# aiola-lab/whisper-medusa

Measured on AMD Instinct MI355X. Metric: decoded_tokens_per_sec, higher is better.
Workload: dtype bf16 + fp16 decoder GEMM operands (one plane; fp32 accumulate)

## Files before the change

### whisper-medusa_amd/csrc/wm_decoder.hip

```cpp
#include "wm_internal.h"
#include <algorithm>
#include <cstdlib>
#include <type_traits>
#include "wm_skinny_gemm.h"
#include "wm_select.h"

__global__ void k_embed(float* __restrict__ h, const bf16_t* __restrict__ tok_emb, const float* __restrict__ pos_emb,
                        const int* __restrict__ base, const int* __restrict__ tok_src, int tok_stride, int use_base_off,
                        int Mper, int d, int V, int Tmax, const int* __restrict__ depth,
                        const int4* __restrict__ rowinfo = nullptr, const int* __restrict__ ids = nullptr, int ids_stride = 0,
                        const float* __restrict__ gnext = nullptr, bf16_t* __restrict__ xo = nullptr, size_t xplane = 0,
                        float2* __restrict__ stats = nullptr, int sld = 0)
{
    const int row = blockIdx.x;
    int s = row / Mper, r = row - s * Mper;
    bool base_row = false;
    int b0;
    if (rowinfo) {
        const int4 ri = rowinfo[row];
        if (ri.w == 0) return;
        s = ri.x; r = ri.y; b0 = ri.z; base_row = ri.w == 1;
    } else {
        b0 = base[s];
    }
// ... 483 lines not shown
                ov[sp] = *reinterpret_cast<const float4*>(&s_part[spc][qr][ch]);
            }
        }
        float Mx = -INFINITY;
#pragma unroll
        for (int sp = 0; sp < WM_XATTN_NS_MAX; ++sp) if (sp < NS) Mx = fmaxf(Mx, ms[sp]);
        float Lt = 0.f; float4 o4 = make_float4(0.f, 0.f, 0.f, 0.f);
#pragma unroll
        for (int sp = 0; sp < WM_XATTN_NS_MAX; ++sp) {
            if (sp < NS) {
                const float e = (ms[sp] == -INFINITY) ? 0.f : __expf(ms[sp] - Mx);
                Lt += ls[sp] * e;
                o4.x += ov[sp].x * e; o4.y += ov[sp].y * e; o4.z += ov[sp].z * e; o4.w += ov[sp].w * e;
            }
        }
        const float inv = vsc / Lt;
        const size_t oi = packed_index(row, hd * 64 + ch, K32);
        act_st4(xout + oi, xout + xplane + oi, make_float4(o4.x * inv, o4.y * inv, o4.z * inv, o4.w * inv));
    }
    TL_END
}


__device__ __forceinline__ void sib_block_pop(float (&tv)[6], int (&ti)[6], float* sv, int* si, int tid, float& mx, int& mi)
{
    const int lane = tid & 63, w = tid >> 6;
    mx = tv[0]; mi = ti[0];
#pragma unroll
    for (int o = 32; o > 0; o >>= 1) {
        const float ov = __shfl_xor(mx, o, 64); const int oi = __shfl_xor(mi, o, 64);
        if (ov > mx || (ov == mx && oi < mi)) { mx = ov; mi = oi; }
    }
    __syncthreads();
    if (lane == 0) { sv[w] = mx; si[w] = mi; }
    __syncthreads();
    mx = sv[0]; mi = si[0];
#pragma unroll
    for (int q = 1; q < 4; ++q) if (sv[q] > mx || (sv[q] == mx && si[q] < mi)) { mx = sv[q]; mi = si[q]; }
    if (ti[0] == mi && mi != 0x7fffffff) {
#pragma unroll
        for (int q = 0; q < 5; ++q) { tv[q] = tv[q + 1]; ti[q] = ti[q + 1]; }
        tv[5] = -INFINITY; ti[5] = 0x7fffffff;
    }
}
__device__ __forceinline__ void sib_insert(float (&tv)[6], int (&ti)[6], float v, int vi)
{
    if (v > tv[5] || (v == tv[5] && vi < ti[5])) {
#pragma unroll
        for (int j = 0; j < 6; ++j)
            if (v > tv[j] || (v == tv[j] && vi < ti[j])) { const float fv = tv[j]; const int fi = ti[j]; tv[j] = v; ti[j] = vi; v = fv; vi = fi; }
    }
}

template <bool NEED_Z, bool TS>
__device__ __forceinline__ void
select1_body(const float* __restrict__ logits, const GenDev& gp, const unsigned char* __restrict__ mask, const float* __restrict__ exppen,
             const int* __restrict__ L, int rps, float* __restrict__ part1, const int4* __restrict__ rowinfo, float2* __restrict__ sibpart,
             const TsDev& ts, int ts_verify)
{
    __shared__ float sv[4]; __shared__ int si[4]; __shared__ float sz[4];
    const int row = blockIdx.y, sp = blockIdx.x;
    int s = row / rps, ri_i = row - s * rps;
    const bool sibrow = sibpart != nullptr && row - s * rps == 1;
    if (rowinfo) {
        const int4 ri = rowinfo[row];
        if (ri.w != 2) return;
        s = ri.x; ri_i = ri.y;
    }
    const int tid = threadIdx.x, lane = tid & 63, w = tid >> 6;
    const int cur_len = L[s];
    const float* x = logits + (size_t)row * gp.Vpad;
    const int per = (gp.V + SEL_SP - 1) / SEL_SP, n0 = sp * per, n1 = min(gp.V, n0 + per);
    int4 rec = make_int4(0, 0, 0, 0);
    if (TS) rec = ts_row_record(gp, ts, ts_verify, s, ri_i, cur_len);
    extern __shared__ unsigned rp_sh[];
    const bool rp = TS && ts.rp != 0;
    if (rp) rp_build(ts, rp_row_prefix(ts, ts_verify, s, ri_i, cur_len), n0, n1, -1, gp.V, rp_sh, tid, 256);
    auto pl = [&](int n) {
        float v = x[n];
        if (rp) v = rp_pen(v, n, n0, ts, rp_sh);
        v = proc_logit(v, n, cur_len, gp, mask, exppen);
        if (TS) v = ts_mask(v, n, rec, gp, ts);
        if (rp && rp_banned(n, n0, gp.V, rp_sh)) v = -INFINITY;
        return v;
    };
    float mx = -INFINITY; int mi = 0x7fffffff;
    if (sibrow) {
        float tv[6]; int ti[6];
#pragma unroll
        for (int j = 0; j < 6; ++j) { tv[j] = -INFINITY; ti[j] = 0x7fffffff; }
        for (int n = n0 + tid; n < n1; n += 256) sib_insert(tv, ti, pl(n), n);
        float2* mine = sibpart + ((size_t)s * SEL_SP + sp) * 6;
        float m0 = -INFINITY; int i0 = 0x7fffffff;
        for (int j = 0; j < 6; ++j) {
            float pm; int pi;
            sib_block_pop(tv, ti, sv, si, tid, pm, pi);
            if (j == 0) { m0 = pm; i0 = pi; }
            if (tid == 0) mine[j] = make_float2(pm, __int_as_float(pi));
        }
        __syncthreads();
        mx = m0; mi = i0;
    } else if (!TS) {
        for (int n = n0 + tid; n < n1; n += 256) {
            const float v = proc_logit(x[n], n, cur_len, gp, mask, exppen);
            if (v > mx || (v == mx && n < mi)) { mx = v; mi = n; }
        }
#pragma unroll
        for (int o = 32; o > 0; o >>= 1) {
            const float ov = __shfl_xor(mx, o, 64); const int oi = __shfl_xor(mi, o, 64);
            if (ov > mx || (ov == mx && oi < mi)) { mx = ov; mi = oi; }
        }
        if (lane == 0) { sv[w] = mx; si[w] = mi; }
        __syncthreads();
        mx = sv[0]; mi = si[0];
#pragma unroll
        for (int k = 1; k < 4; ++k) if (sv[k] > mx || (sv[k] == mx && si[k] < mi)) { mx = sv[k]; mi = si[k]; }
    }
    if (TS) {
        float mt = -INFINITY, ms = -INFINITY; int it = 0x7fffffff, is = 0x7fffffff;
        for (int n = n0 + tid; n < n1; n += 256) {
            const float v = pl(n);
            if (n < ts.tb) { if (v > mt || (v == mt && n < it)) { mt = v; it = n; } }
            else if (v > ms || (v == ms && n < is)) { ms = v; is = n; }
        }
        block_argmax(mt, it, sv, si, tid);
        block_argmax(ms, is, sv, si, tid);
        float zt = 0.f, zs = 0.f, zs1 = 0.f;
        for (int n = (NEED_Z ? n0 : max(n0, ts.tb)) + tid; n < n1; n += 256) {
            const float v = pl(n);
            if (v == -INFINITY) continue;
            if (n < ts.tb) zt += expf((v - mt) * gp.inv_temp);
            else { if (NEED_Z) zs += expf((v - ms) * gp.inv_temp); zs1 += expf(v - ms); }
        }
        zt = block_sum(zt, sz, tid); zs = block_sum(zs, sz, tid); zs1 = block_sum(zs1, sz, tid);
        if (tid == 0) {
            float* o = part1 + ((size_t)row * SEL_SP + sp) * 4;
            o[0] = mt; o[1] = __int_as_float(it); o[2] = zt;
            float* q = ts.part1t + ((size_t)row * SEL_SP + sp) * 4;
            q[0] = ms; q[1] = __int_as_float(is); q[2] = zs; q[3] = zs1;
        }
        return;
    }
    float z = 0.f;
    if (NEED_Z && mx != -INFINITY)
        for (int n = n0 + tid; n < n1; n += 256) {
            const float v = proc_logit(x[n], n, cur_len, gp, mask, exppen);
            z += (v == -INFINITY) ? 0.f : expf((v - mx) * gp.inv_temp);
        }
    z = wave_sum(z);
    if (lane == 0) sz[w] = z;
    __syncthreads();
    if (tid == 0) {
        float* o = part1 + ((size_t)row * SEL_SP + sp) * 4;
        o[0] = mx; o[1] = __int_as_float(mi); o[2] = (sz[0] + sz[1]) + (sz[2] + sz[3]);
    }
}

template <bool NEED_Z = true>
__global__ void __launch_bounds__(256)
k_select1(const float* __restrict__ logits, GenDev gp, const unsigned char* __restrict__ mask, const float* __restrict__ exppen,
          const int* __restrict__ L, int rps, float* __restrict__ part1, const int4* __restrict__ rowinfo = nullptr,
          float2* __restrict__ sibpart = nullptr)
{
    select1_body<NEED_Z, false>(logits, gp, mask, exppen, L, rps, part1, rowinfo, sibpart, TsDev{}, 0);
}
template <bool NEED_Z>
__global__ void __launch_bounds__(256)
k_select1_ts(const float* __restrict__ logits, GenDev gp, const unsigned char* __restrict__ mask, const float* __restrict__ exppen,
             const int* __restrict__ L, int rps, float* __restrict__ part1, const int4* __restrict__ rowinfo, float2* __restrict__ sibpart,
             TsDev ts, int ts_verify)
{
    select1_body<NEED_Z, true>(logits, gp, mask, exppen, L, rps, part1, rowinfo, sibpart, ts, ts_verify);
}

template <bool TS>
__device__ __forceinline__ void
select2_body(const float* __restrict__ logits, const GenDev& gp, const unsigned char* __restrict__ mask, const float* __restrict__ exppen,
             const int* __restrict__ L, const int* __restrict__ cand, int rps, int out_row0, const float* __restrict__ part1,
             float* __restrict__ part2, int* __restrict__ amax, float* __restrict__ pc, const TreeDev* __restrict__ tree,
             const int4* __restrict__ rowinfo, const TsDev& ts)
{
    __shared__ float sh[4];
    const int row = blockIdx.y, sp = blockIdx.x;
    int s = row / rps, i = row - s * rps;
    if (rowinfo) {
        const int4 ri = rowinfo[row];
        if (ri.w != 2) return;
        s = ri.x; i = ri.y;
    }
    const int tid = threadIdx.x, lane = tid & 63, w = tid >> 6;
    const int cur_len = L[s];
    const float* x = logits + (size_t)row * gp.Vpad;
    const float* p1 = part1 + (size_t)row * SEL_SP * 4;
    float mx = -INFINITY; int mi = 0x7fffffff;
    float invz;
    int4 rec = make_int4(0, 0, 0, 0); int forced = 0;
    if (TS) {
        const TsSel f = ts_finish(p1, ts.part1t + (size_t)row * SEL_SP * 4, gp.inv_temp);
        mx = f.mx; mi = f.mi; invz = 1.0f / f.z; forced = f.forced;
        rec = ts_row_record(gp, ts, 1, s, i, cur_len);
    } else {
#pragma unroll
        for (int k = 0; k < SEL_SP; ++k) {
            const float v = p1[4 * k]; const int idx = __float_as_int(p1[4 * k + 1]);
            if (v > mx || (v == mx && idx < mi)) { mx = v; mi = idx; }
        }
        float z = 0.f;
#pragma unroll
        for (int k = 0; k < SEL_SP; ++k) {
            const float v = p1[4 * k];
            z += (v == -INFINITY) ? 0.f : p1[4 * k + 2] * expf((v - mx) * gp.inv_temp);
        }
        invz = 1.0f / z;
    }
    const int per = (gp.V + SEL_SP - 1) / SEL_SP, n0 = sp * per, n1 = min(gp.V, n0 + per);
    extern __shared__ unsigned rp_sh[];
    const bool rp = TS && ts.rp != 0;
    const int probe = (TS && i + 1 < rps) ? cand[s * WM_CAND_STRIDE + i + 1] : -1;
    if (rp) rp_build(ts, rp_row_prefix(ts, 1, s, i, cur_len), n0, n1, probe, gp.V, rp_sh, tid, 256);
    auto pl = [&](int n) {
        float v = x[n];
        if (rp) v = rp_pen(v, n, n0, ts, rp_sh);
        v = proc_logit(v, n, cur_len, gp, mask, exppen);
        if (TS) { v = ts_mask(v, n, rec, gp, ts); if (forced && n < ts.tb) v = -INFINITY; }
        if (rp && rp_banned(n, n0, gp.V, rp_sh)) v = -INFINITY;
        return v;
    };
    auto pl_probe = [&](int n) {
        float v = x[n];
        if (rp && (rp_sh[0] & 1u)) v = rp_penalise(v, ts.rp_pen);
        v = proc_logit(v, n, cur_len, gp, mask, exppen);
        if (TS) { v = ts_mask(v, n, rec, gp, ts); if (forced && n < ts.tb) v = -INFINITY; }
        if (rp && (rp_sh[0] & 2u)) v = -INFINITY;
        return v;
    };
    float hs = 0.f;
    for (int n = n0 + tid; n < n1; n += 256) {
        const float v = pl(n);
        const float p = (v == -INFINITY) ? 0.f : expf((v - mx) * gp.inv_temp) * invz;
        hs += p * logf(p + 1e-5f);
    }
    hs = wave_sum(hs);
    if (lane == 0) sh[w] = hs;
    __syncthreads();
    if (tid == 0) {
        const int orow = out_row0 + row;
        part2[(size_t)orow * SEL_SP + sp] = (sh[0] + sh[1]) + (sh[2] + sh[3]);
        if (sp == 0) {
            amax[orow] = mi;
            if (TS) ts.forced[orow] = forced;
            if (tree) {
                if (i == 0) pc[out_row0 + s * rps] = 0.f;
                for (int j = 0; j < 4; ++j) {
                    const int ch = tree->children[i][j];
                    if (ch < 0) break;
                    const int c = cand[s * WM_CAND_STRIDE + ch];
                    const float vc = proc_logit(x[c], c, cur_len, gp, mask, exppen);
                    pc[out_row0 + s * rps + ch] = (vc == -INFINITY) ? 0.f : expf((vc - mx) * gp.inv_temp) * invz;
                }
            } else {
                float pcv = 0.f;
                if (i + 1 < rps) {
                    const int c = cand[s * WM_CAND_STRIDE + i + 1];
                    const float vc = pl_probe(c);
// ... 38 lines not shown
    const int row = blockIdx.x * blockDim.x + threadIdx.x;
    if (row >= nrows) return;
    const TsSel f = ts_finish(part1 + (size_t)row * SEL_SP * 4, ts.part1t + (size_t)row * SEL_SP * 4, 1.0f);
    amax[out_row0 + row] = f.mi;
    ts.forced[out_row0 + row] = f.forced;
}

__global__ void k_rows_take_carried(float* __restrict__ dst, const float* __restrict__ keep, const int* __restrict__ carry, int d, int M,
                                    const int* __restrict__ done)
{
    if (done && *done) return;
    const int m = blockIdx.x;
    if (m >= M || !carry[m]) return;
    const float4* sp = reinterpret_cast<const float4*>(keep + (size_t)m * d);
    float4* dp = reinterpret_cast<float4*>(dst + (size_t)m * d);
    for (int j = threadIdx.x; j < (d >> 2); j += blockDim.x) dp[j] = sp[j];
}

template <bool TS>
__device__ __forceinline__ void
cand_fin_body(const float* __restrict__ part1, const GenDev& gp, int* __restrict__ amax, int* __restrict__ cand, const float2* __restrict__ sibpart,
              const TsDev& ts)
{
    __shared__ float sv[4]; __shared__ int si[4];
    const int s = blockIdx.x, tid = threadIdx.x, rps = gp.K + 1;
    if (tid < rps) {
        const float* p1 = part1 + (size_t)(s * rps + tid) * SEL_SP * 4;
        float mx = -INFINITY; int mi = 0x7fffffff;
        if (TS) mi = ts_finish(p1, ts.part1t + (size_t)(s * rps + tid) * SEL_SP * 4, 1.0f).mi;
        else
            for (int k = 0; k < SEL_SP; ++k) {
                const float v = p1[4 * k]; const int idx = __float_as_int(p1[4 * k + 1]);
                if (v > mx || (v == mx && idx < mi)) { mx = v; mi = idx; }
            }
        amax[s * rps + tid] = mi;
        cand[s * WM_CAND_STRIDE + tid] = mi;
    }
    if (TS) {
        __syncthreads();
        if (tid == 0 && ts.on) {
            int4 st = ts.st[s];
            const int len = ts.L[s];
            for (int i = 0; i < rps; ++i) {
                st = ts_fold(st, cand[s * WM_CAND_STRIDE + i], ts.tb);
                ts.ver[s * WM_CAND_STRIDE + i] = ts_record(st, len + i + 1, gp.begin, ts.tb, gp.V, ts.mit);
            }
        }
    }
    if (gp.sib <= 0 || sibpart == nullptr) return;
    float tv[6]; int ti[6];
#pragma unroll
    for (int j = 0; j < 6; ++j) { tv[j] = -INFINITY; ti[j] = 0x7fffffff; }
    if (tid < SEL_SP * 6) {
        const float2 p = sibpart[(size_t)s * SEL_SP * 6 + tid];
        tv[0] = p.x; ti[0] = __float_as_int(p.y);
    }
    for (int j = 0; j <= gp.sib; ++j) {
        float mx; int mi;
        sib_block_pop(tv, ti, sv, si, tid, mx, mi);
        if (tid == 0 && j > 0) cand[s * WM_CAND_STRIDE + gp.K + j] = (mi == 0x7fffffff) ? -1 : mi;
    }
}

__global__ void __launch_bounds__(256)
k_cand_fin(const float* __restrict__ part1, GenDev gp, int* __restrict__ amax, int* __restrict__ cand, const float2* __restrict__ sibpart)
{
    cand_fin_body<false>(part1, gp, amax, cand, sibpart, TsDev{});
}
__global__ void __launch_bounds__(256)
k_cand_fin_ts(const float* __restrict__ part1, GenDev gp, int* __restrict__ amax, int* __restrict__ cand, const float2* __restrict__ sibpart,
              TsDev ts)
{
    cand_fin_body<true>(part1, gp, amax, cand, sibpart, ts);
}

__global__ void __launch_bounds__(256)
k_step_begin(const int* __restrict__ carry, const int* __restrict__ L, const int* __restrict__ kvlen, const int* __restrict__ finished,
             int4* __restrict__ rowinfo, int4* __restrict__ sinfo, int* __restrict__ steprows, int rps, int B, int Rmax)
{
    __shared__ int s_start[1025];
    if (threadIdx.x == 0) {
        int acc = 0;
        for (int s = 0; s < B; ++s) { s_start[s] = acc; acc += finished[s] ? 0 : (carry[s] ? rps : 1); }
        s_start[B] = acc;
        steprows[0] = acc; steprows[1] = (acc + 15) >> 4;
        if (acc > 0) steprows[2] += 1;
    }
    __syncthreads();
    const int nrows = s_start[B];
    for (int s = threadIdx.x; s < B; s += blockDim.x) {
        const int m = carry[s] ? 1 : 0, cnt = finished[s] ? 0 : (m ? rps : 1), pb = m ? L[s] : kvlen[s], r0 = s_start[s];
        sinfo[s] = make_int4(r0, cnt, pb, m);
        for (int r = 0; r < cnt; ++r) rowinfo[r0 + r] = make_int4(s, r, pb, m ? 2 : 1);
    }
    for (int row = nrows + threadIdx.x; row < Rmax; row += blockDim.x) rowinfo[row] = make_int4(0, 0, 0, 0);
}

template <bool TS>
__device__ __forceinline__ void
accept_body(const GenDev& gp, const int* __restrict__ cand, const int* __restrict__ amax, const float* __restrict__ pc,
            const float* __restrict__ part2, int* __restrict__ ids, int* __restrict__ L, int* __restrict__ kvlen,
            int* __restrict__ finished, int* __restrict__ niter, long long* __restrict__ hist, int* __restrict__ done, int B,
            int* __restrict__ carry, const float* __restrict__ hf, float* __restrict__ hf_keep, int d,
            int* __restrict__ hostflags, const float* __restrict__ hb, float* __restrict__ hb_keep,
            const int4* __restrict__ sinfo, int* __restrict__ sel_src, int* __restrict__ sel_n, int* __restrict__ sel_base, const TsDev& ts)
{
    const int s = blockIdx.x, lane = threadIdx.x;
    if (finished[s]) { if (sel_n && lane == 0) sel_n[s] = 0; return; }
    const int K = gp.K, rps = K + 1;
    const int row0 = sinfo ? sinfo[s].x : s * rps;
    if (sinfo != nullptr && sinfo[s].w == 0) {
        const float4* srcp = reinterpret_cast<const float4*>(hf + (size_t)row0 * d);
        float4* dstp = reinterpret_cast<float4*>(hf_keep + (size_t)s * d);
        for (int j = lane; j < (d >> 2); j += 64) dstp[j] = srcp[j];
        if (hb) {
            const float4* bs = reinterpret_cast<const float4*>(hb + (size_t)row0 * d);
            float4* bd = reinterpret_cast<float4*>(hb_keep + (size_t)s * d);
            for (int j = lane; j < (d >> 2); j += 64) bd[j] = bs[j];
// ... 37 lines not shown
    if (do_carry) {
        const float4* srcp = reinterpret_cast<const float4*>(hf + (size_t)(row0 + crow) * d);
        float4* dstp = reinterpret_cast<float4*>(hf_keep + (size_t)s * d);
        for (int j = lane; j < (d >> 2); j += 64) dstp[j] = srcp[j];
        if (hb) {
            const float4* bs = reinterpret_cast<const float4*>(hb + (size_t)(row0 + crow) * d);
            float4* bd = reinterpret_cast<float4*>(hb_keep + (size_t)s * d);
            for (int j = lane; j < (d >> 2); j += 64) bd[j] = bs[j];
        }
    }
    if (sel_n != nullptr && lane < 16) sel_src[s * 16 + lane] = (lane == 1 && sib_row >= 0) ? sib_row : lane;
    if (lane == 0) {
        const int Ln = Lcur + n_emit;
        if (TS && ts.on) {
            int4 st = ts.st[s];
            for (int j = 0; j < n_emit; ++j) st = ts_fold(st, (a == 0 && j == 1) ? amax[row0] : cand[s * WM_CAND_STRIDE + j], ts.tb);
            ts.st[s] = st;
        }
        L[s] = Ln;
        kvlen[s] = (a == 0 && sib_row < 0) ? Lcur + 1 : (do_carry ? Ln : Lcur + a);
        if (carry) carry[s] = do_carry ? 1 : 0;
        if (sel_n != nullptr) { sel_n[s] = sib_row >= 0 ? 2 : 0; sel_base[s] = Lcur; }
        if (sib_row >= 0) atomicAdd(reinterpret_cast<unsigned long long*>(hist + 17), 1ull);
        niter[s] += 1;
        atomicAdd(reinterpret_cast<unsigned long long*>(hist + a), 1ull);
        atomicAdd(reinterpret_cast<unsigned long long*>(hist + 16), (unsigned long long)n_emit);
        const bool fin = hit_eos || Ln >= gp.max_length || Ln + K >= gp.hard_max_length;
        if (fin) {
            finished[s] = 1;
            if (atomicAdd(done + 1, 1) == B - 1) done[0] = 1;
        }
        if (hostflags) { hostflags[0] = do_carry ? 1 : 0; hostflags[1] = fin ? 1 : 0; }
    }
}

#define WM_ACCEPT_PARAMS                                                                                                        \
    GenDev gp, const int* __restrict__ cand, const int* __restrict__ amax, const float* __restrict__ pc, const float* __restrict__ part2,  \
    int* __restrict__ ids, int* __restrict__ L, int* __restrict__ kvlen, int* __restrict__ finished, int* __restrict__ niter,             \
    long long* __restrict__ hist, int* __restrict__ done, int B, int* __restrict__ carry, const float* __restrict__ hf,                    \
    float* __restrict__ hf_keep, int d, int* __restrict__ hostflags, const float* __restrict__ hb, float* __restrict__ hb_keep
__global__ void k_accept(WM_ACCEPT_PARAMS, const int4* __restrict__ sinfo = nullptr, int* __restrict__ sel_src = nullptr,
                         int* __restrict__ sel_n = nullptr, int* __restrict__ sel_base = nullptr)
{
    accept_body<false>(gp, cand, amax, pc, part2, ids, L, kvlen, finished, niter, hist, done, B, carry, hf, hf_keep, d, hostflags, hb, hb_keep,
                       sinfo, sel_src, sel_n, sel_base, TsDev{});
}
__global__ void k_accept_ts(WM_ACCEPT_PARAMS, const int4* __restrict__ sinfo, int* __restrict__ sel_src, int* __restrict__ sel_n,
                            int* __restrict__ sel_base, TsDev ts)
{
    accept_body<true>(gp, cand, amax, pc, part2, ids, L, kvlen, finished, niter, hist, done, B, carry, hf, hf_keep, d, hostflags, hb, hb_keep,
                      sinfo, sel_src, sel_n, sel_base, ts);
}
#undef WM_ACCEPT_PARAMS

__global__ void __launch_bounds__(256)
// ... 90 lines not shown
    const bool hit_eos = __ballot(lane < n_emit && tok == gp.eos) != 0ull;
    const bool do_carry = carry != nullptr && a > 0;
    const int n_keep = (a == 0) ? 1 : (do_carry ? a + 1 : a);
    const int my_src = (lane < n_keep) ? tree->retrieve[best][lane] : lane;
    if (lane < 16) sel_src[s * 16 + lane] = my_src;
    const bool moved = __ballot(lane < n_keep && my_src != lane) != 0ull;
    if (do_carry) {
        const int nd = tree->retrieve[best][a];
        const float4* srcp = reinterpret_cast<const float4*>(hf + (size_t)(s * tn + nd) * d);
        float4* dstp = reinterpret_cast<float4*>(hf_keep + (size_t)s * d);
        for (int j = lane; j < (d >> 2); j += 64) dstp[j] = srcp[j];
        if (hb) {
            const float4* bs = reinterpret_cast<const float4*>(hb + (size_t)(s * tn + nd) * d);
            float4* bd = reinterpret_cast<float4*>(hb_keep + (size_t)s * d);
            for (int j = lane; j < (d >> 2); j += 64) bd[j] = bs[j];
        }
    }
    if (lane == 0) {
        const int Ln = Lcur + n_emit;
        sel_n[s] = moved ? n_keep : 0; sel_base[s] = Lcur;
        L[s] = Ln;
        kvlen[s] = Lcur + n_keep;
        if (carry) carry[s] = do_carry ? 1 : 0;
        niter[s] += 1;
        atomicAdd(reinterpret_cast<unsigned long long*>(hist + a), 1ull);
        atomicAdd(reinterpret_cast<unsigned long long*>(hist + 16), (unsigned long long)n_emit);
        const bool fin = hit_eos || Ln >= gp.max_length || Ln + K >= gp.hard_max_length;
        if (fin) {
            finished[s] = 1;
            if (atomicAdd(done + 1, 1) == B - 1) done[0] = 1;
        }
        if (hostflags) { hostflags[0] = do_carry ? 1 : 0; hostflags[1] = fin ? 1 : 0; }
    }
}

__global__ void __launch_bounds__(256)
k_kv_compact(bf16_t* __restrict__ kc, bf16_t* __restrict__ vc, const int* __restrict__ sel_src, const int* __restrict__ sel_n,
             const int* __restrict__ sel_base, int H, int Tal, int maxB)
{
    const int hd = blockIdx.x, s = blockIdx.y, slot = blockIdx.z;
    const int n = sel_n[s];
    if (n == 0) return;
    const int base = sel_base[s];
    const int i = threadIdx.x >> 4, q = threadIdx.x & 15;
    const size_t off = (((size_t)slot * maxB + s) * H + hd) * (size_t)Tal * 64;
    bf16_t* kp = kc + off; bf16_t* vp = vc + off;
    uint2 kv = make_uint2(0u, 0u); bf16_t vv[4] = {0, 0, 0, 0};
    const bool act = i < n;
    if (act) {
        const int src = base + sel_src[s * 16 + i];
        kv = *reinterpret_cast<const uint2*>(kp + (size_t)src * 64 + q * 4);
#pragma unroll
        for (int j = 0; j < 4; ++j) vv[j] = vp[vfrag_index(src, q * 4 + j)];
    }
    __syncthreads();
// ... 765 lines not shown
```

### whisper-medusa_amd/csrc/wm_engine.hip

```cpp
#include <algorithm>
#include <cmath>
#include <cstdlib>
#include <cstring>
#include "wm_select.h"

static thread_local std::string g_create_err;

static inline int rup(int x, int m) { return (x + m - 1) / m * m; }

template <class T>
static hipError_t dev_alloc(T** p, size_t n, hipStream_t st)
{
    hipError_t e = hipMalloc(reinterpret_cast<void**>(p), std::max<size_t>(n, 1) * sizeof(T));
    if (e != hipSuccess) return e;
    return hipMemsetAsync(*p, 0, std::max<size_t>(n, 1) * sizeof(T), st);
}

extern "C" int wm_abi_version(void) { return WM_ABI_VERSION; }
extern "C" int wm_build_act_fp16(void) { return WM_ACT_PLANES == 1 ? 1 : 0; }

extern "C" const char* wm_last_error(const wm_ctx* ctx) { return ctx ? ctx->err.c_str() : g_create_err.c_str(); }

extern "C" void wm_destroy(wm_ctx* ctx)
{
// ... 216 lines not shown
    CREATE_HIP(dev_alloc(&ctx->ts.part1t, RW * 16 * 4, st));
    CREATE_HIP(dev_alloc(&ctx->ts.forced, RW + B, st));
    CREATE_HIP(dev_alloc(&ctx->samp.part, RW * 16 * 8, st));
    CREATE_HIP(dev_alloc(&ctx->samp.val, RW + B, st));
    CREATE_HIP(dev_alloc(&ctx->samp_keys, std::max<size_t>(B, 16), st));
    CREATE_HIP(dev_alloc(&ctx->samp.fv, std::max<size_t>(B, 16) * ctx->Vpad, st));
    CREATE_HIP(dev_alloc(&ctx->samp.thr, RW + B, st));
    CREATE_HIP(dev_alloc(&ctx->samp.kept, RW + B, st));
    ctx->samp.top_k = 0; ctx->samp.top_p = 1.0f; ctx->samp.min_p = 0.0f;
    CREATE_HIP(dev_alloc(&ctx->lang_ids, WM_LANG_MAX, st));
    CREATE_HIP(dev_alloc(&ctx->lang_out, std::max<size_t>(B, 16), st));
    const size_t Tids = ctx->Tal;
    CREATE_HIP(dev_alloc(&ctx->ids, B * Tids, st));
    CREATE_HIP(dev_alloc(&ctx->L, B, st));
    CREATE_HIP(dev_alloc(&ctx->kvlen, B, st));
    CREATE_HIP(dev_alloc(&ctx->finished, B, st));
    CREATE_HIP(dev_alloc(&ctx->cand, B * WM_CAND_STRIDE, st));
    CREATE_HIP(dev_alloc(&ctx->niter, B, st));
    CREATE_HIP(dev_alloc(&ctx->hist, 32, st));
    CREATE_HIP(dev_alloc(&ctx->supmask, (size_t)ctx->Vpad, st));
    CREATE_HIP(dev_alloc(&ctx->exppen, Tids + 1, st));
    CREATE_HIP(dev_alloc(&ctx->tap_tok, 16, st));
    CREATE_HIP(dev_alloc(&ctx->done, 4, st));
    CREATE_HIP(hipHostMalloc(reinterpret_cast<void**>(&ctx->hostflags), 64, hipHostMallocMapped));
    CREATE_HIP(hipHostGetDevicePointer(reinterpret_cast<void**>(&ctx->hostflags_dev), ctx->hostflags, 0));
    ctx->hostflags[0] = ctx->hostflags[1] = 0;
    if (ctx->ln_fold && wm_dec_fold_init(ctx) != WM_OK) { g_create_err = "wm_create: " + ctx->err; wm_destroy(ctx); return WM_ERR_HIP; }
    CREATE_HIP(hipStreamSynchronize(st));
#undef CREATE_HIP
    *out = ctx;
    return WM_OK;
}

extern "C" int wm_sync(wm_ctx* ctx) { WM_HIP(hipSetDevice(ctx->device)); WM_HIP(hipStreamSynchronize(ctx->stream)); return WM_OK; }

extern "C" int64_t wm_resample_len(int64_t n_in, int sr_in, int sr_out) { return wm_enc_resample_len((long)n_in, sr_in, sr_out); }

extern "C" int wm_resample(wm_ctx* ctx, const float* in, int B, int channels, int n_in, int sr_in, int sr_out, float* out)
{
    if (!ctx || !in || !out) return WM_ERR_ARG;
    WM_HIP(hipSetDevice(ctx->device));
    return wm_enc_resample(ctx, in, B, channels, n_in, sr_in, sr_out, out);
}

extern "C" int wm_logmel(wm_ctx* ctx, const float* wav, int B, int n_samples, float* feats)
{
    if (!ctx || !wav || !feats) return WM_ERR_ARG;
    WM_HIP(hipSetDevice(ctx->device));
    return wm_enc_logmel(ctx, wav, B, n_samples, feats);
// ... 215 lines not shown
        for (int i = 0; i < P; ++i) ids[(size_t)b * Tids + i] = row[i];
    }
    WM_HIP(hipMemcpyAsync(ctx->ids, ids.data(), ids.size() * sizeof(int), hipMemcpyHostToDevice, st));
    WM_HIP(hipMemcpyAsync(ctx->L, L.data(), B * sizeof(int), hipMemcpyHostToDevice, st));
    WM_HIP(hipMemcpyAsync(ctx->kvlen, zero.data(), B * sizeof(int), hipMemcpyHostToDevice, st));
    WM_HIP(hipMemcpyAsync(ctx->finished, zero.data(), B * sizeof(int), hipMemcpyHostToDevice, st));
    WM_HIP(hipMemcpyAsync(ctx->niter, zero.data(), B * sizeof(int), hipMemcpyHostToDevice, st));
    WM_HIP(hipMemsetAsync(ctx->hist, 0, 32 * sizeof(long long), st));
    WM_HIP(hipMemsetAsync(ctx->done, 0, 4 * sizeof(int), st));
    WM_HIP(hipMemsetAsync(ctx->carry, 0, ctx->maxB * sizeof(int), st));
    WM_HIP(hipMemsetAsync(ctx->steprows, 0, 4 * sizeof(int), st));
    ctx->use_done = true;
    std::vector<int4> tst(B, make_int4(0, 0, -1, 0));
    if (ts.on) {
        for (int b = 0; b < B; ++b)
            for (int i = std::max(g.begin, 0); i < P; ++i) tst[b] = ts_fold(tst[b], ids[(size_t)b * Tids + i], ts.tb);
        WM_HIP(hipMemcpyAsync(ctx->ts.st, tst.data(), B * sizeof(int4), hipMemcpyHostToDevice, st));
    }
    if (beam) {
        if (int rc = wm_beam_seed_table(ctx, bd)) return rc;
        if (int rc = wm_beam_expand(ctx, G, nbeam)) return rc;
    }
    WM_HIP(hipStreamSynchronize(st));
    ctx->hostflags[0] = 0; ctx->hostflags[1] = 0;
    ctx->began = true; ctx->first_done = false; ctx->iters = 0; ctx->ms_decode = 0.f; ctx->graph_replays = 0;
    return WM_OK;
}

static int count_unfinished(wm_ctx* ctx, int* n)
{
    std::vector<int> f(ctx->Bdec);
    WM_HIP(hipMemcpyAsync(f.data(), ctx->finished, ctx->Bdec * sizeof(int), hipMemcpyDeviceToHost, ctx->stream));
    WM_HIP(hipStreamSynchronize(ctx->stream));
    int c = 0;
    for (int v : f) c += v ? 0 : 1;
    *n = c;
    return WM_OK;
}

static int capture_graph(wm_ctx* ctx, hipGraphExec_t* out, int (*body)(wm_ctx*, int))
{
    hipStream_t st = ctx->stream;
    hipGraph_t gr = nullptr;
    *out = nullptr;
    if (hipStreamBeginCapture(st, hipStreamCaptureModeThreadLocal) != hipSuccess) { (void)hipGetLastError(); return WM_OK; }
    const int rc = body(ctx, 1);
    const hipError_t e2 = hipStreamEndCapture(st, &gr);
    if (rc == WM_OK && e2 == hipSuccess && gr) {
        hipGraphExec_t ex = nullptr;
        if (hipGraphInstantiate(&ex, gr, nullptr, nullptr, 0) == hipSuccess) *out = ex;
    }
    if (gr) hipGraphDestroy(gr);
    (void)hipGetLastError();
    return WM_OK;
}

extern "C" int wm_decode_run(wm_ctx* ctx, int max_iters, int* n_unfinished)
{
    if (!ctx) return WM_ERR_ARG;
    WM_HIP(hipSetDevice(ctx->device));
    if (!ctx->began) { ctx->err = "wm_decode_run: call wm_decode_begin first"; return WM_ERR_STATE; }
    hipStream_t st = ctx->stream;
    const bool use_graph = std::getenv("WM_NO_GRAPH") == nullptr;
    DecGraphSlot& gs = ctx->beam.on ? ctx->graphs_beam : ctx->graphs_plain;
    int left = 0, done = 0;
    int rc = count_unfinished(ctx, &left);
    if (rc) return rc;
    WM_HIP(hipEventRecord(ctx->ev0, st));
    if (ctx->host_carry) {
        while (left > 0 && done < max_iters) {
            if (!ctx->first_done) {
                const int p_last = wm_dec_prompt_prefix(ctx, ctx->gp.P);
                if (p_last < 1) return WM_ERR_HIP;
                rc = wm_dec_iteration(ctx, p_last);
                if (rc) return rc;
                ctx->first_done = true;
            } else {
                const bool need_base = ctx->hostflags[0] == 0;
                const bool warm = ctx->iters >= 2;
                if (need_base) {
                    if (use_graph && warm && !gs.base) { rc = capture_graph(ctx, &gs.base, wm_dec_iter_base); if (rc) return rc; }
                    if (use_graph && gs.base) WM_HIP(hipGraphLaunch(gs.base, st));
                    else { rc = wm_dec_iter_base(ctx, 1); if (rc) return rc; }
                }
                if (use_graph && warm && !gs.step) { rc = capture_graph(ctx, &gs.step, wm_dec_iter_rest); if (rc) return rc; }
                if (use_graph && gs.step) { WM_HIP(hipGraphLaunch(gs.step, st)); ctx->graph_replays++; }
                else { rc = wm_dec_iter_rest(ctx, 1); if (rc) return rc; }
            }
            WM_HIP(hipStreamSynchronize(st));
            ctx->iters++; done++;
            left = ctx->hostflags[1] ? 0 : 1;
        }
    } else {
        const int poll = 4;
        while (left > 0 && done < max_iters) {
            const int burst = std::min(poll, max_iters - done);
            for (int i = 0; i < burst; ++i) {
                if (!ctx->first_done) {
                    const int p_last = wm_dec_prompt_prefix(ctx, ctx->gp.P);
                    if (p_last < 1) return WM_ERR_HIP;
                    rc = wm_dec_iteration(ctx, p_last);
                    if (rc) return rc;
                    ctx->first_done = true;
                } else {
                    int (*body)(wm_ctx*, int) = ctx->step_flow ? wm_dec_step : wm_dec_iteration;
                    if (use_graph && ctx->iters >= 2 && !gs.step) { rc = capture_graph(ctx, &gs.step, body); if (rc) return rc; }
                    if (use_graph && gs.step) { WM_HIP(hipGraphLaunch(gs.step, st)); ctx->graph_replays++; }
                    else { rc = body(ctx, 1); if (rc) return rc; }
                }
                ctx->iters++; done++;
            }
            rc = count_unfinished(ctx, &left);
// ... 278 lines not shown
```

### whisper-medusa_amd/csrc/wm_internal.h

```cpp
#pragma once
#include <hip/hip_runtime.h>
#include <algorithm>
#include <cstring>
#include <string>
#include <vector>
#include "../../include/wm.h"
#include "wm_common.h"

#define WM_HIP(expr)                                                                        \
    do {                                                                                    \
        hipError_t _e = (expr);                                                             \
        if (_e != hipSuccess) {                                                             \
            ctx->err = std::string(#expr) + ": " + hipGetErrorString(_e);                   \
            return WM_ERR_HIP;                                                              \
        }                                                                                   \
    } while (0)

struct EncLayerW {
    const float *ln1_w, *ln1_b, *qkv_b, *out_b, *ln2_w, *ln2_b, *fc1_b, *fc2_b;
    const bf16_t *qkv_w, *out_w, *fc1_w, *fc2_w;
    const unsigned char *qkv_w8 = nullptr, *fc1_w8 = nullptr;
    const float *qkv_ws = nullptr, *fc1_ws = nullptr;
};
struct DecLayerW {
// ... 193 lines not shown
    int Benc = 0;

    float *h = nullptr, *hblk = nullptr, *hf = nullptr, *qbuf = nullptr;
    float *hb_keep = nullptr;
    float *hf_cur = nullptr, *hf_keep = nullptr;
    int* carry = nullptr;
    int4* rowinfo = nullptr;
    int4* sinfo = nullptr;
    int* steprows = nullptr;
    bool step_flow = false;
    int tn = 0, tp = 0;
    TreeDev tree_host{};
    TreeDev* tree = nullptr;
    TreeDev* sibtree = nullptr;
    int sib_cfg = 0;
    float2* sibpart = nullptr;
    const unsigned long long* cur_anc = nullptr;
    int *sel_src = nullptr, *sel_n = nullptr, *sel_base = nullptr;
    bool fuse = true;
    bool host_carry = false;
    float* rs_table = nullptr; int rs_og = 0, rs_nw = 0, rs_width = 0;
    bool dev_carry = false;
    int *hostflags = nullptr, *hostflags_dev = nullptr;
    bf16_t *xbuf = nullptr, *fbuf = nullptr, *ybuf = nullptr;
    bf16_t* xn = nullptr; float2* lnstats = nullptr; float* foldv = nullptr;
    bool ln_fold = false;
    float *cml = nullptr, *co = nullptr;
    int* ticket = nullptr;
    float* logits = nullptr;
    int* amax = nullptr; float *pc = nullptr;
    float *part1 = nullptr, *part2 = nullptr;

    int *ids = nullptr, *L = nullptr, *kvlen = nullptr, *finished = nullptr, *cand = nullptr, *niter = nullptr;
    long long* hist = nullptr;
    unsigned char* supmask = nullptr;
    float* exppen = nullptr;
    int* tap_tok = nullptr;
    int* done = nullptr;
    bool use_done = false;
    GenDev gp{};
    TsDev ts{};
    wm_repeat_params rep{1.0f, 0};
    bool samp_set_on = false; float samp_set_temp = 1.0f; uint64_t samp_set_seed = 0; std::vector<uint64_t> samp_set_keys;
    bool samp_filter_on = false; wm_sample_filter samp_filter{0, 1.0f, 0.0f};
    SampDev samp{};
    unsigned long long* samp_keys = nullptr;
// ... 16 lines not shown
    hipEvent_t ev0 = nullptr, ev1 = nullptr;
    bool prefetch = true;
    float ms_logmel = 0.f, ms_encode = 0.f, ms_decode = 0.f;

    struct wm_align_state* align = nullptr;
    struct wm_score_state* score = nullptr;
    bool replay = false;
};

long wm_enc_resample_len(long n_in, int sr_in, int sr_out);
int wm_enc_resample(wm_ctx* ctx, const float* in, int B, int channels, int n_in, int sr_in, int sr_out, float* out);
int wm_enc_logmel(wm_ctx* ctx, const float* wav, int B, int n_samples, float* feats);
int wm_enc_encode(wm_ctx* ctx, const float* feats, int B);
int wm_enc_set_output(wm_ctx* ctx, const float* hidden, int B);
int wm_enc_quant_cross_kv(wm_ctx* ctx, int B);
int wm_dec_stage_layers(wm_ctx* ctx, int b0, int nb, int Mper, int mode );
int wm_dec_stage_final(wm_ctx* ctx, int b0, int nb, int Mper, int mode, int medusa);
int wm_dec_stage_heads(wm_ctx* ctx, int nsel, int sel_mul, int sel_off, int medusa);
int wm_dec_pass(wm_ctx* ctx, int b0, int nb, int Mper, int mode, int medusa, int all_rows);
int wm_dec_iteration(wm_ctx* ctx, int Mper_base);
int wm_dec_prompt_prefix(wm_ctx* ctx, int P);
int wm_dec_iter_base(wm_ctx* ctx, int Mper_base);
int wm_dec_iter_rest(wm_ctx* ctx, int Mper_base);
int wm_dec_step(wm_ctx* ctx, int);
int wm_dec_profile(wm_ctx* ctx, int kernel, int rows, int reps, float* ms, double* bytes);
int wm_dec_fold_init(wm_ctx* ctx);
struct wm_replay_hooks {
    int (*layer)(wm_ctx*, int, int, int, void*) = nullptr;
    int (*tile)(wm_ctx*, int, int, void*) = nullptr;
    void* arg = nullptr;
};
int wm_dec_replay(wm_ctx* ctx, int b0, int nb, const int32_t* tokens, int Tmax, const int32_t* lens, int npos, int n_layers, const wm_replay_hooks& hooks);
int wm_replay_check(wm_ctx* ctx, const char* who, int B, int Tmax, const int32_t* lens, const int32_t* n_prompt, int min_prompt);
int wm_sample_launch(wm_ctx* ctx, const GenDev& gp, const TsDev& ts, const SampDev& sd, const int* pos, int nrows, int out_row0, int tap);
int wm_beam_check(wm_ctx* ctx, const char* who, const wm_beam_params* bp);
int wm_beam_begin(wm_ctx* ctx, const wm_beam_params& bp, int G, const GenDev& g, bool kv, const float* init_scores, int len0, BeamDev* out);
int wm_beam_seed_table(wm_ctx* ctx, const BeamDev& bd);
int wm_beam_step(wm_ctx* ctx, const GenDev& gp, const TsDev& ts, const BeamDev& bd, bool kv);
int wm_beam_expand(wm_ctx* ctx, int G, int n);
int wm_beam_compact(wm_ctx* ctx);
void wm_beam_free(wm_ctx* ctx);
int wm_seq_bias_begin(wm_ctx* ctx, const char* who, const wm_gen_params* gp, SeqBiasDev* out);
int wm_seq_bias_launch(wm_ctx* ctx, const SeqBiasDev& sb, const int* ids, int ids_stride, const int* lens, int len_cap, int nrows);
void wm_seq_bias_free(wm_ctx* ctx);
void wm_align_free(wm_ctx* ctx);
void wm_score_free(wm_ctx* ctx);
// ... 10 lines not shown
```

### whisper-medusa_amd/csrc/wm_select.h

```cpp
#pragma once
#include "wm_internal.h"

#define SEL_SP 16

__device__ __forceinline__ float proc_logit(float x, int n, int cur_len, const GenDev& gp, const unsigned char* mask,
                                            const float* exppen)
{
    if (n == gp.eos && gp.exp_start >= 0 && cur_len > gp.exp_start) x += fabsf(x) * exppen[cur_len];
    const unsigned char mk = mask[n];
    if ((mk & 1) || ((mk & 2) && cur_len == gp.begin)) x = -INFINITY;
    return x;
}

__device__ __forceinline__ float ts_mask(float v, int n, int4 rec, const GenDev& gp, const TsDev& ts)
{
    if (n == ts.nots) return -INFINITY;
    if (n >= ts.tb) return (n < rec.x || n > rec.y) ? -INFINITY : v;
    return ((rec.z & 2) || ((rec.z & 1) && n < gp.eos)) ? -INFINITY : v;
}
__device__ __forceinline__ int4 ts_row_record(const GenDev& gp, const TsDev& ts, int ts_verify, int s, int i, int cur_len)
{
    if (!ts.on) return make_int4(0, 0, 0, 0);
    return ts_verify ? ts.ver[s * WM_CAND_STRIDE + i] : ts_record(ts.st[s], cur_len, gp.begin, ts.tb, gp.V, ts.mit);
}

struct RpPre { const int* pre; int len; const int* ext; int next; };
__host__ __device__ __forceinline__ int rp_words(int V) { return V / (32 * SEL_SP) + 3; }
static inline size_t rp_lds_bytes(const TsDev& ts, int V) { return ts.rp ? (size_t)(4 + 2 * rp_words(V)) * sizeof(unsigned) : 0; }
__device__ __forceinline__ int rp_tok(const RpPre& p, int j) { return j < p.len ? p.pre[j] : p.ext[j - p.len]; }
__device__ __forceinline__ void rp_build(const TsDev& ts, const RpPre& p, int n0, int n1, int probe, int V, unsigned* sh, int tid, int nthr)
{
    const int W = rp_words(V);
    for (int k = tid; k < 4 + 2 * W; k += nthr) sh[k] = 0u;
    __syncthreads();
// ... 82 lines not shown
```

Measured before the change: 1560.

## Cache select logits in registers, parallelize sibling top-k, add host spin-poll

The select kernels now load each thread's slice of logits and mask into registers once and reuse the processed values across the argmax, normalizer and entropy passes instead of re-reading global memory. The sibling top-6 reduction now works per wave and ranks by counting, replacing the chain of block-wide barrier pops. The host-carry decode loop spin-polls a coherent host-mapped iteration counter, falling back to stream synchronize after a timeout, to cut per-iteration sync latency. This adds register pressure (13 values per thread) and burns a CPU core while spinning.

Result: no change. 1572 (median of 6 runs) (+0.7%).

```diff
diff --git a/whisper-medusa_amd/csrc/wm_decoder.hip b/whisper-medusa_amd/csrc/wm_decoder.hip
--- a/whisper-medusa_amd/csrc/wm_decoder.hip
+++ b/whisper-medusa_amd/csrc/wm_decoder.hip
@@ -529,26 +529,31 @@
 }
 
 
-__device__ __forceinline__ void sib_block_pop(float (&tv)[6], int (&ti)[6], float* sv, int* si, int tid, float& mx, int& mi)
-{
-    const int lane = tid & 63, w = tid >> 6;
+__device__ __forceinline__ void sib_wave_pop(float (&tv)[6], int (&ti)[6], float& mx, int& mi)
+{
     mx = tv[0]; mi = ti[0];
 #pragma unroll
     for (int o = 32; o > 0; o >>= 1) {
         const float ov = __shfl_xor(mx, o, 64); const int oi = __shfl_xor(mi, o, 64);
         if (ov > mx || (ov == mx && oi < mi)) { mx = ov; mi = oi; }
     }
-    __syncthreads();
-    if (lane == 0) { sv[w] = mx; si[w] = mi; }
-    __syncthreads();
-    mx = sv[0]; mi = si[0];
-#pragma unroll
-    for (int q = 1; q < 4; ++q) if (sv[q] > mx || (sv[q] == mx && si[q] < mi)) { mx = sv[q]; mi = si[q]; }
     if (ti[0] == mi && mi != 0x7fffffff) {
 #pragma unroll
         for (int q = 0; q < 5; ++q) { tv[q] = tv[q + 1]; ti[q] = ti[q + 1]; }
         tv[5] = -INFINITY; ti[5] = 0x7fffffff;
     }
+}
+__device__ __forceinline__ int sib_place(const float2* pairs, int n, float v, int vi, int& real)
+{
+    int place = 0;
+    real = 0;
+    for (int q = 0; q < n; ++q) {
+        const float2 e = pairs[q];
+        const int ei = __float_as_int(e.y);
+        place += (e.x > v || (e.x == v && ei < vi)) ? 1 : 0;
+        real += (ei != 0x7fffffff) ? 1 : 0;
+    }
+    return place;
 }
 __device__ __forceinline__ void sib_insert(float (&tv)[6], int (&ti)[6], float v, int vi)
 {
@@ -575,43 +580,72 @@
         s = ri.x; ri_i = ri.y;
     }
     const int tid = threadIdx.x, lane = tid & 63, w = tid >> 6;
-    const int cur_len = L[s];
     const float* x = logits + (size_t)row * gp.Vpad;
     const int per = (gp.V + SEL_SP - 1) / SEL_SP, n0 = sp * per, n1 = min(gp.V, n0 + per);
+    const bool fits = per <= 256 * SEL_NJ;
+    float rx[SEL_NJ]; unsigned char rm[SEL_NJ];
+    if (fits) {
+#pragma unroll
+        for (int j = 0; j < SEL_NJ; ++j) {
+            const int nc = min(n0 + tid + 256 * j, gp.V - 1);
+            rx[j] = x[nc]; rm[j] = mask[nc];
+        }
+    }
+    const int cur_len = L[s];
     int4 rec = make_int4(0, 0, 0, 0);
     if (TS) rec = ts_row_record(gp, ts, ts_verify, s, ri_i, cur_len);
     extern __shared__ unsigned rp_sh[];
     const bool rp = TS && ts.rp != 0;
     if (rp) rp_build(ts, rp_row_prefix(ts, ts_verify, s, ri_i, cur_len), n0, n1, -1, gp.V, rp_sh, tid, 256);
-    auto pl = [&](int n) {
-        float v = x[n];
+    auto pl = [&](float v, unsigned char mk, int n) {
         if (rp) v = rp_pen(v, n, n0, ts, rp_sh);
-        v = proc_logit(v, n, cur_len, gp, mask, exppen);
+        v = proc_logit_mk(v, n, cur_len, gp, mk, exppen);
         if (TS) v = ts_mask(v, n, rec, gp, ts);
         if (rp && rp_banned(n, n0, gp.V, rp_sh)) v = -INFINITY;
         return v;
     };
+    float rv[SEL_NJ];
+    if (fits) {
+#pragma unroll
+        for (int j = 0; j < SEL_NJ; ++j) {
+            const int n = n0 + tid + 256 * j;
+            rv[j] = (n < n1) ? pl(rx[j], rm[j], n) : -INFINITY;
+        }
+    }
+    auto each = [&](int from, auto&& f) {
+        if (fits && from == n0) {
+#pragma unroll
+            for (int j = 0; j < SEL_NJ; ++j) { const int n = n0 + tid + 256 * j; if (n < n1) f(rv[j], n); }
+        } else
+            for (int n = from + tid; n < n1; n += 256) f(pl(x[n], mask[n], n), n);
+    };
     float mx = -INFINITY; int mi = 0x7fffffff;
     if (sibrow) {
+        __shared__ float2 swp[24];
         float tv[6]; int ti[6];
 #pragma unroll
         for (int j = 0; j < 6; ++j) { tv[j] = -INFINITY; ti[j] = 0x7fffffff; }
-        for (int n = n0 + tid; n < n1; n += 256) sib_insert(tv, ti, pl(n), n);
-        float2* mine = sibpart + ((size_t)s * SEL_SP + sp) * 6;
-        float m0 = -INFINITY; int i0 = 0x7fffffff;
+        each(n0, [&](float v, int n) { sib_insert(tv, ti, v, n); });
+#pragma unroll
         for (int j = 0; j < 6; ++j) {
             float pm; int pi;
-            sib_block_pop(tv, ti, sv, si, tid, pm, pi);
-            if (j == 0) { m0 = pm; i0 = pi; }
-            if (tid == 0) mine[j] = make_float2(pm, __int_as_float(pi));
+            sib_wave_pop(tv, ti, pm, pi);
+            if (lane == 0) swp[w * 6 + j] = make_float2(pm, __int_as_float(pi));
         }
         __syncthreads();
-        mx = m0; mi = i0;
+        if (tid < 24) {
+            const float2 me = swp[tid];
+            float2* mine = sibpart + ((size_t)s * SEL_SP + sp) * 6;
+            int real;
+            const int place = sib_place(swp, 24, me.x, __float_as_int(me.y), real);
+            if (place < 6 && __float_as_int(me.y) != 0x7fffffff) mine[place] = me;
+            if (tid < 6 && tid >= real) mine[tid] = make_float2(-INFINITY, __int_as_float(0x7fffffff));
+            if (place == 0) { sv[0] = me.x; si[0] = __float_as_int(me.y); }
+        }
+        __syncthreads();
+        mx = sv[0]; mi = si[0];
     } else if (!TS) {
-        for (int n = n0 + tid; n < n1; n += 256) {
-            const float v = proc_logit(x[n], n, cur_len, gp, mask, exppen);
-            if (v > mx || (v == mx && n < mi)) { mx = v; mi = n; }
-        }
+        each(n0, [&](float v, int n) { if (v > mx || (v == mx && n < mi)) { mx = v; mi = n; } });
 #pragma unroll
         for (int o = 32; o > 0; o >>= 1) {
             const float ov = __shfl_xor(mx, o, 64); const int oi = __shfl_xor(mi, o, 64);
@@ -625,20 +659,18 @@
     }
     if (TS) {
         float mt = -INFINITY, ms = -INFINITY; int it = 0x7fffffff, is = 0x7fffffff;
-        for (int n = n0 + tid; n < n1; n += 256) {
-            const float v = pl(n);
+        each(n0, [&](float v, int n) {
             if (n < ts.tb) { if (v > mt || (v == mt && n < it)) { mt = v; it = n; } }
             else if (v > ms || (v == ms && n < is)) { ms = v; is = n; }
-        }
+        });
         block_argmax(mt, it, sv, si, tid);
         block_argmax(ms, is, sv, si, tid);
         float zt = 0.f, zs = 0.f, zs1 = 0.f;
-        for (int n = (NEED_Z ? n0 : max(n0, ts.tb)) + tid; n < n1; n += 256) {
-            const float v = pl(n);
-            if (v == -INFINITY) continue;
+        each(NEED_Z ? n0 : max(n0, ts.tb), [&](float v, int n) {
+            if (v == -INFINITY) return;
             if (n < ts.tb) zt += expf((v - mt) * gp.inv_temp);
             else { if (NEED_Z) zs += expf((v - ms) * gp.inv_temp); zs1 += expf(v - ms); }
-        }
+        });
         zt = block_sum(zt, sz, tid); zs = block_sum(zs, sz, tid); zs1 = block_sum(zs1, sz, tid);
         if (tid == 0) {
             float* o = part1 + ((size_t)row * SEL_SP + sp) * 4;
@@ -650,10 +682,7 @@
     }
     float z = 0.f;
     if (NEED_Z && mx != -INFINITY)
-        for (int n = n0 + tid; n < n1; n += 256) {
-            const float v = proc_logit(x[n], n, cur_len, gp, mask, exppen);
-            z += (v == -INFINITY) ? 0.f : expf((v - mx) * gp.inv_temp);
-        }
+        each(n0, [&](float v, int) { z += (v == -INFINITY) ? 0.f : expf((v - mx) * gp.inv_temp); });
     z = wave_sum(z);
     if (lane == 0) sz[w] = z;
     __syncthreads();
@@ -696,8 +725,18 @@
         s = ri.x; i = ri.y;
     }
     const int tid = threadIdx.x, lane = tid & 63, w = tid >> 6;
+    const float* x = logits + (size_t)row * gp.Vpad;
+    const int per = (gp.V + SEL_SP - 1) / SEL_SP, n0 = sp * per, n1 = min(gp.V, n0 + per);
+    const bool fits = per <= 256 * SEL_NJ;
+    float rx[SEL_NJ]; unsigned char rm[SEL_NJ];
+    if (fits) {
+#pragma unroll
+        for (int j = 0; j < SEL_NJ; ++j) {
+            const int nc = min(n0 + tid + 256 * j, gp.V - 1);
+            rx[j] = x[nc]; rm[j] = mask[nc];
+        }
+    }
     const int cur_len = L[s];
-    const float* x = logits + (size_t)row * gp.Vpad;
     const float* p1 = part1 + (size_t)row * SEL_SP * 4;
     float mx = -INFINITY; int mi = 0x7fffffff;
     float invz;
@@ -720,15 +759,13 @@
         }
         invz = 1.0f / z;
     }
-    const int per = (gp.V + SEL_SP - 1) / SEL_SP, n0 = sp * per, n1 = min(gp.V, n0 + per);
     extern __shared__ unsigned rp_sh[];
     const bool rp = TS && ts.rp != 0;
     const int probe = (TS && i + 1 < rps) ? cand[s * WM_CAND_STRIDE + i + 1] : -1;
     if (rp) rp_build(ts, rp_row_prefix(ts, 1, s, i, cur_len), n0, n1, probe, gp.V, rp_sh, tid, 256);
-    auto pl = [&](int n) {
-        float v = x[n];
+    auto pl = [&](float v, unsigned char mk, int n) {
         if (rp) v = rp_pen(v, n, n0, ts, rp_sh);
-        v = proc_logit(v, n, cur_len, gp, mask, exppen);
+        v = proc_logit_mk(v, n, cur_len, gp, mk, exppen);
         if (TS) { v = ts_mask(v, n, rec, gp, ts); if (forced && n < ts.tb) v = -INFINITY; }
         if (rp && rp_banned(n, n0, gp.V, rp_sh)) v = -INFINITY;
         return v;
@@ -742,11 +779,15 @@
         return v;
     };
     float hs = 0.f;
-    for (int n = n0 + tid; n < n1; n += 256) {
-        const float v = pl(n);
+    auto term = [&](float v) {
         const float p = (v == -INFINITY) ? 0.f : expf((v - mx) * gp.inv_temp) * invz;
         hs += p * logf(p + 1e-5f);
-    }
+    };
+    if (fits) {
+#pragma unroll
+        for (int j = 0; j < SEL_NJ; ++j) { const int n = n0 + tid + 256 * j; if (n < n1) term(pl(rx[j], rm[j], n)); }
+    } else
+        for (int n = n0 + tid; n < n1; n += 256) term(pl(x[n], mask[n], n));
     hs = wave_sum(hs);
     if (lane == 0) sh[w] = hs;
     __syncthreads();
@@ -831,7 +872,6 @@
 cand_fin_body(const float* __restrict__ part1, const GenDev& gp, int* __restrict__ amax, int* __restrict__ cand, const float2* __restrict__ sibpart,
               const TsDev& ts)
 {
-    __shared__ float sv[4]; __shared__ int si[4];
     const int s = blockIdx.x, tid = threadIdx.x, rps = gp.K + 1;
     if (tid < rps) {
         const float* p1 = part1 + (size_t)(s * rps + tid) * SEL_SP * 4;
@@ -857,17 +897,16 @@
         }
     }
     if (gp.sib <= 0 || sibpart == nullptr) return;
-    float tv[6]; int ti[6];
-#pragma unroll
-    for (int j = 0; j < 6; ++j) { tv[j] = -INFINITY; ti[j] = 0x7fffffff; }
+    __shared__ float2 sw[SEL_SP * 6];
+    float2 me = make_float2(-INFINITY, __int_as_float(0x7fffffff));
+    if (tid < SEL_SP * 6) { me = sibpart[(size_t)s * SEL_SP * 6 + tid]; sw[tid] = me; }
+    __syncthreads();
     if (tid < SEL_SP * 6) {
-        const float2 p = sibpart[(size_t)s * SEL_SP * 6 + tid];
-        tv[0] = p.x; ti[0] = __float_as_int(p.y);
-    }
-    for (int j = 0; j <= gp.sib; ++j) {
-        float mx; int mi;
-        sib_block_pop(tv, ti, sv, si, tid, mx, mi);
-        if (tid == 0 && j > 0) cand[s * WM_CAND_STRIDE + gp.K + j] = (mi == 0x7fffffff) ? -1 : mi;
+        const int mi = __float_as_int(me.y);
+        int real;
+        const int place = sib_place(sw, SEL_SP * 6, me.x, mi, real);
+        if (mi != 0x7fffffff && place >= 1 && place <= gp.sib) cand[s * WM_CAND_STRIDE + gp.K + place] = mi;
+        if (tid >= 1 && tid <= gp.sib && tid >= real) cand[s * WM_CAND_STRIDE + gp.K + tid] = -1;
     }
 }
 
@@ -903,6 +942,12 @@
         for (int r = 0; r < cnt; ++r) rowinfo[r0 + r] = make_int4(s, r, pb, m ? 2 : 1);
     }
     for (int row = nrows + threadIdx.x; row < Rmax; row += blockDim.x) rowinfo[row] = make_int4(0, 0, 0, 0);
+}
+
+__device__ __forceinline__ void accept_publish(int* __restrict__ hostflags, bool do_carry, bool fin, int iteration)
+{
+    hostflags[0] = do_carry ? 1 : 0; hostflags[1] = fin ? 1 : 0;
+    __hip_atomic_store(hostflags + 2, iteration, __ATOMIC_RELEASE, __HIP_MEMORY_SCOPE_SYSTEM);
 }
 
 template <bool TS>
@@ -986,7 +1031,8 @@
         if (carry) carry[s] = do_carry ? 1 : 0;
         if (sel_n != nullptr) { sel_n[s] = sib_row >= 0 ? 2 : 0; sel_base[s] = Lcur; }
         if (sib_row >= 0) atomicAdd(reinterpret_cast<unsigned long long*>(hist + 17), 1ull);
-        niter[s] += 1;
+        const int it = niter[s] + 1;
+        niter[s] = it;
         atomicAdd(reinterpret_cast<unsigned long long*>(hist + a), 1ull);
         atomicAdd(reinterpret_cast<unsigned long long*>(hist + 16), (unsigned long long)n_emit);
         const bool fin = hit_eos || Ln >= gp.max_length || Ln + K >= gp.hard_max_length;
@@ -994,7 +1040,7 @@
             finished[s] = 1;
             if (atomicAdd(done + 1, 1) == B - 1) done[0] = 1;
         }
-        if (hostflags) { hostflags[0] = do_carry ? 1 : 0; hostflags[1] = fin ? 1 : 0; }
+        if (hostflags) accept_publish(hostflags, do_carry, fin, it);
     }
 }
 
@@ -1131,7 +1177,8 @@
         L[s] = Ln;
         kvlen[s] = Lcur + n_keep;
         if (carry) carry[s] = do_carry ? 1 : 0;
-        niter[s] += 1;
+        const int it = niter[s] + 1;
+        niter[s] = it;
         atomicAdd(reinterpret_cast<unsigned long long*>(hist + a), 1ull);
         atomicAdd(reinterpret_cast<unsigned long long*>(hist + 16), (unsigned long long)n_emit);
         const bool fin = hit_eos || Ln >= gp.max_length || Ln + K >= gp.hard_max_length;
@@ -1139,7 +1186,7 @@
             finished[s] = 1;
             if (atomicAdd(done + 1, 1) == B - 1) done[0] = 1;
         }
-        if (hostflags) { hostflags[0] = do_carry ? 1 : 0; hostflags[1] = fin ? 1 : 0; }
+        if (hostflags) accept_publish(hostflags, do_carry, fin, it);
     }
 }
 
diff --git a/whisper-medusa_amd/csrc/wm_engine.hip b/whisper-medusa_amd/csrc/wm_engine.hip
--- a/whisper-medusa_amd/csrc/wm_engine.hip
+++ b/whisper-medusa_amd/csrc/wm_engine.hip
@@ -1,4 +1,5 @@
 #include <algorithm>
+#include <chrono>
 #include <cmath>
 #include <cstdlib>
 #include <cstring>
@@ -262,9 +263,9 @@
     CREATE_HIP(dev_alloc(&ctx->exppen, Tids + 1, st));
     CREATE_HIP(dev_alloc(&ctx->tap_tok, 16, st));
     CREATE_HIP(dev_alloc(&ctx->done, 4, st));
-    CREATE_HIP(hipHostMalloc(reinterpret_cast<void**>(&ctx->hostflags), 64, hipHostMallocMapped));
+    CREATE_HIP(hipHostMalloc(reinterpret_cast<void**>(&ctx->hostflags), 64, hipHostMallocMapped | hipHostMallocCoherent));
     CREATE_HIP(hipHostGetDevicePointer(reinterpret_cast<void**>(&ctx->hostflags_dev), ctx->hostflags, 0));
-    ctx->hostflags[0] = ctx->hostflags[1] = 0;
+    ctx->hostflags[0] = ctx->hostflags[1] = ctx->hostflags[2] = 0;
     if (ctx->ln_fold && wm_dec_fold_init(ctx) != WM_OK) { g_create_err = "wm_create: " + ctx->err; wm_destroy(ctx); return WM_ERR_HIP; }
     CREATE_HIP(hipStreamSynchronize(st));
 #undef CREATE_HIP
@@ -526,7 +527,10 @@
         if (int rc = wm_beam_expand(ctx, G, nbeam)) return rc;
     }
     WM_HIP(hipStreamSynchronize(st));
-    ctx->hostflags[0] = 0; ctx->hostflags[1] = 0;
+    ctx->hostflags[0] = 0; ctx->hostflags[1] = 0; ctx->hostflags[2] = 0;
+    const char* hp = std::getenv("WM_HOST_POLL");
+    ctx->host_poll = host_carry && !(hp && hp[0] == '0');
+    ctx->host_wait_ms = ctx->host_launch_ms = 0.0; ctx->host_poll_timeouts = 0;
     ctx->began = true; ctx->first_done = false; ctx->iters = 0; ctx->ms_decode = 0.f; ctx->graph_replays = 0;
     return WM_OK;
 }
@@ -556,6 +560,29 @@
     }
     if (gr) hipGraphDestroy(gr);
     (void)hipGetLastError();
+    return WM_OK;
+}
+
+using wm_clock = std::chrono::steady_clock;
+static double wm_ms_between(wm_clock::time_point a, wm_clock::time_point b) { return std::chrono::duration<double, std::milli>(b - a).count(); }
+static bool wm_wait_iteration(const int* word, int want)
+{
+    const wm_clock::time_point t0 = wm_clock::now();
+    for (;;) {
+        for (int i = 0; i < 64; ++i) {
+            if (__atomic_load_n(word, __ATOMIC_ACQUIRE) == want) return true;
+#if defined(__x86_64__) || defined(__i386__)
+            __builtin_ia32_pause();
+#endif
+        }
+        if (wm_ms_between(t0, wm_clock::now()) > 50.0) return false;
+    }
+}
+
+extern "C" int wm_get_host_loop(wm_ctx* ctx, double out[4])
+{
+    if (!ctx || !out) return WM_ERR_ARG;
+    out[0] = ctx->host_wait_ms; out[1] = ctx->host_launch_ms; out[2] = ctx->host_carry ? (double)ctx->iters : 0.0; out[3] = (double)ctx->host_poll_timeouts;
     return WM_OK;
 }
 
@@ -573,6 +600,7 @@
     WM_HIP(hipEventRecord(ctx->ev0, st));
     if (ctx->host_carry) {
         while (left > 0 && done < max_iters) {
+            const wm_clock::time_point t_launch = wm_clock::now();
             if (!ctx->first_done) {
                 const int p_last = wm_dec_prompt_prefix(ctx, ctx->gp.P);
                 if (p_last < 1) return WM_ERR_HIP;
@@ -591,7 +619,12 @@
                 if (use_graph && gs.step) { WM_HIP(hipGraphLaunch(gs.step, st)); ctx->graph_replays++; }
                 else { rc = wm_dec_iter_rest(ctx, 1); if (rc) return rc; }
             }
-            WM_HIP(hipStreamSynchronize(st));
+            const wm_clock::time_point t_wait = wm_clock::now();
+            if (ctx->host_poll && !wm_wait_iteration(ctx->hostflags + 2, (int)ctx->iters + 1)) {
+                ctx->host_poll = false; ctx->host_poll_timeouts++;
+            }
+            if (!ctx->host_poll) WM_HIP(hipStreamSynchronize(st));
+            ctx->host_launch_ms += wm_ms_between(t_launch, t_wait); ctx->host_wait_ms += wm_ms_between(t_wait, wm_clock::now());
             ctx->iters++; done++;
             left = ctx->hostflags[1] ? 0 : 1;
         }
diff --git a/whisper-medusa_amd/csrc/wm_internal.h b/whisper-medusa_amd/csrc/wm_internal.h
--- a/whisper-medusa_amd/csrc/wm_internal.h
+++ b/whisper-medusa_amd/csrc/wm_internal.h
@@ -239,6 +239,9 @@
     float* rs_table = nullptr; int rs_og = 0, rs_nw = 0, rs_width = 0;
     bool dev_carry = false;
     int *hostflags = nullptr, *hostflags_dev = nullptr;
+    bool host_poll = false;
+    double host_wait_ms = 0.0, host_launch_ms = 0.0;
+    int host_poll_timeouts = 0;
     bf16_t *xbuf = nullptr, *fbuf = nullptr, *ybuf = nullptr;
     bf16_t* xn = nullptr; float2* lnstats = nullptr; float* foldv = nullptr;
     bool ln_fold = false;
@@ -301,6 +304,7 @@
 int wm_dec_prompt_prefix(wm_ctx* ctx, int P);
 int wm_dec_iter_base(wm_ctx* ctx, int Mper_base);
 int wm_dec_iter_rest(wm_ctx* ctx, int Mper_base);
+extern "C" int wm_get_host_loop(wm_ctx* ctx, double out[4]);
 int wm_dec_step(wm_ctx* ctx, int);
 int wm_dec_profile(wm_ctx* ctx, int kernel, int rows, int reps, float* ms, double* bytes);
 int wm_dec_fold_init(wm_ctx* ctx);
diff --git a/whisper-medusa_amd/csrc/wm_select.h b/whisper-medusa_amd/csrc/wm_select.h
--- a/whisper-medusa_amd/csrc/wm_select.h
+++ b/whisper-medusa_amd/csrc/wm_select.h
@@ -2,14 +2,18 @@
 #include "wm_internal.h"
 
 #define SEL_SP 16
+#define SEL_NJ 13
 
+__device__ __forceinline__ float proc_logit_mk(float x, int n, int cur_len, const GenDev& gp, unsigned char mk, const float* exppen)
+{
+    if (n == gp.eos && gp.exp_start >= 0 && cur_len > gp.exp_start) x += fabsf(x) * exppen[cur_len];
+    if ((mk & 1) || ((mk & 2) && cur_len == gp.begin)) x = -INFINITY;
+    return x;
+}
 __device__ __forceinline__ float proc_logit(float x, int n, int cur_len, const GenDev& gp, const unsigned char* mask,
                                             const float* exppen)
 {
-    if (n == gp.eos && gp.exp_start >= 0 && cur_len > gp.exp_start) x += fabsf(x) * exppen[cur_len];
-    const unsigned char mk = mask[n];
-    if ((mk & 1) || ((mk & 2) && cur_len == gp.begin)) x = -INFINITY;
-    return x;
+    return proc_logit_mk(x, n, cur_len, gp, mask[n], exppen);
 }
 
 __device__ __forceinline__ float ts_mask(float v, int n, int4 rec, const GenDev& gp, const TsDev& ts)
```
